# xbpeng/DeepTerrainRL

Measured on AMD Instinct MI355X. Metric: env-steps/sec (batched rollout) dog/slopes_mixed, higher is better.
Workload: dtype f64

## Files before the change

### deepterrainrl_amd/csrc/dtrl_kernel.h

```cpp
#pragma once
#include "dtrl_types.h"
#include <cmath>

#if defined(__HIPCC__)
#include <hip/hip_runtime.h>
#define DTRL_HD __host__ __device__
#define DTRL_HD_INLINE __host__ __device__ __forceinline__
#define DTRL_HD_NOINLINE __host__ __device__ __attribute__((noinline))
#else
#define DTRL_HD
#define DTRL_HD_INLINE inline
#define DTRL_HD_NOINLINE inline
#endif

#if defined(__HIP_DEVICE_COMPILE__)
#define LANES_BEGIN { const int lane = static_cast<int>(threadIdx.x);
#define LANES_END } ::dtrl::env_sync();
#else
#define LANES_BEGIN for (int lane = 0; lane < ::dtrl::kGroup; ++lane) {
#define LANES_END }
#endif

#if defined(__HIP_DEVICE_COMPILE__) && defined(DTRL_PROFILE)
#define PROF_T0() const unsigned long long prof_t0_ = __builtin_readcyclecounter()
#define PROF_ADD(ws, id) do { if (threadIdx.x == 0) (ws).prof[id] += __builtin_readcyclecounter() - prof_t0_; } while (0)
#define PROF_NOW() __builtin_readcyclecounter()
#define PROF_ADD_SINCE(ws, id, t0) do { if (threadIdx.x == 0) (ws).prof[id] += __builtin_readcyclecounter() - (t0); } while (0)
#define PROF_COUNT(ws, id) do { if (threadIdx.x == 0) (ws).prof[id] += 1; } while (0)
#else
#define PROF_T0() do {} while (0)
#define PROF_ADD(ws, id) do {} while (0)
#define PROF_NOW() 0ull
#define PROF_ADD_SINCE(ws, id, t0) do { (void)(t0); } while (0)
#define PROF_COUNT(ws, id) do {} while (0)
#endif

namespace dtrl {

#if defined(__HIP_DEVICE_COMPILE__)
#ifndef DTRL_WAVE_SYNC
#define DTRL_WAVE_SYNC 1
#endif
#if DTRL_WAVE_SYNC && !defined(__GFX9__)
#error "env_sync(): wavefront-scope fences are only a barrier when the 64-thread workgroup is ONE wavefront (GFX9 / CDNA: wave64). On a wave32 target the workgroup is two waves: build with -DDTRL_WAVE_SYNC=0 (ADVICE r4)"
#endif
__device__ __forceinline__ void env_sync()
{
#if DTRL_WAVE_SYNC
	static_assert(kGroup == 64, "env_sync(): one wavefront per env");
	__builtin_amdgcn_fence(__ATOMIC_RELEASE, "wavefront");
	__builtin_amdgcn_wave_barrier();
	__builtin_amdgcn_fence(__ATOMIC_ACQUIRE, "wavefront");
#else
	__syncthreads();
#endif
}
#else
inline void env_sync() {}
#endif

enum ProfSection { kProfFK, kProfMass, kProfBias, kProfFact, kProfDetect, kProfRows, kProfFsub, kProfDelassus, kProfPgs, kProfFinish, kProfCtrl, kProfAction, kProfFrameIO, kProfTotal, kProfRowsSum, kProfSubsteps, kProfP1, kProfP2, kProfP3, kProfP4, kProfR0, kProfR1_6, kProfR7_12, kProfR13_18, kProfR19_24, kProfT0, kProfT1_6, kProfT7_12, kProfT13_18, kProfT19_24, kProfNNConv, kProfNNFcTerr, kProfNNRest, kProfNNEvals, kProfC_Fsm, kProfC_Feedback, kProfC_PdSetup, kProfC_PdSolve, kProfC_Grav, kProfC_Tail, kProfMax };

struct HotModel {
	int32_t L, D, char_type, n_pairs;
	int32_t warm_start;
	int32_t parent[kMaxL], depth[kMaxL], col[kMaxL];
	int8_t pair_l[kMaxPairs], pair_k[kMaxPairs];
	alignas(4) int8_t path[kMaxL][kMaxDepth];
	uint32_t sub_mask[kMaxL];
	uint32_t anc_mask[kMaxL];
	real attach[kMaxL][2], lim_lo[kMaxL], lim_hi[kMaxL];
	real body_attach[kMaxL][2];
	real mass[kMaxL], inertia[kMaxL], sub_mass[kMaxL];
	int32_t n_cpairs;
	int8_t cp_a[kMaxCP], cp_b[kMaxCP];
	float cp_half[kMaxL][2];
	float cp_root_bt[2];
};

struct DevBuffers {
	EnvState* st;
	GroundRec* gr;
	EnvStatus* status;
	real* poli_state;
	real* tup_s0;
	real* tup_a;
	real* nn_out;
	float* tuple_rows;
	uint32_t* tuple_flags;
	int32_t* tuple_env;
	int32_t* tuple_count;
	int32_t tuple_cap;
	int32_t S, A, W;
	int32_t model_D;
	int32_t model_topo;
	unsigned long long* prof;
	const int32_t* env_list;
	int32_t reset_listed;
	GroundGen* gen;
	const TerrainCfg* tcfg;
	DistRec* dist_ring; int32_t* dist_count; int32_t dist_cap;
	const GroundRec* gr_stage; int32_t* stage_slot;
	const float* weights;
	const real* in_off; const real* in_scale; const real* out_off; const real* out_scale;
	NetDesc net;
};

constexpr int kZStride = kMaxD + 1;
struct WSBase {
	HotModel M;
	EnvState st;
	real phi[kMaxL], cs[kMaxL], sn[kMaxL], w[kMaxL];
	real px[kMaxL], py[kMaxL], cx[kMaxL], cy[kMaxL];
	real vpx[kMaxL], vpy[kMaxL], vcx[kMaxL], vcy[kMaxL];
	real fx[kMaxL], fy[kMaxL], fn[kMaxL];
	real mcx[kMaxL], mcy[kMaxL], Io[kMaxL];
	real sfs[3][kMaxL];
	union {
		struct { real bx[kMaxL], by[kMaxL], ux[kMaxL], uy[kMaxL], gx[kMaxL], gy[kMaxL]; };
		struct { real sm[kMaxL], smx[kMaxL], smy[kMaxL], sI[kMaxL]; };
	};
	real dinv[kMaxD];
	real b[kMaxD];
	real u[kMaxD];
	int32_t R, n_pts_active;
	int32_t row_kind[kMaxRows], row_link[kMaxRows];
	int8_t row_link2[kMaxRows];
	real row_x[kMaxRows], row_y[kMaxRows], row_dx[kMaxRows], row_dy[kMaxRows], row_tgt[kMaxRows];
	uint16_t row_id[kMaxRows];
	real wv[kMaxRows], rinv[kMaxRows];
	real dl;
	union {
		real Z[kMaxRows + 1][kZStride];
		struct {
			real z0_[kZStride];
			real basis[kMaxD][4];
			real tau_g[kMaxD];
			real kpv[kMaxD], kdv[kMaxD], kdm[kMaxD], perr[kMaxD], verr[kMaxD];
		};
	};
	real red[8];
	int32_t flag_update_action, flag_new_cycle, flag_misc;
	int32_t cost;
#if defined(DTRL_PROFILE)
	unsigned long long prof[kProfMax];
#endif
};
struct WSRef : WSBase {
	real H[kMaxD][kMaxD + 1];
	union {
		real A[kMaxRows][kMaxRows + 1];
		struct {
			real pt_x[kMaxPts], pt_y[kMaxPts], pt_depth[kMaxPts], pt_nx[kMaxPts], pt_ny[kMaxPts];
			int32_t pt_active[kMaxPts];
		};
	};
};
constexpr int kPackedA = kMaxRows * (kMaxRows + 1) / 2;
constexpr int kMassTab = kMaxL * (kMaxDepth + 2);
struct WSFast : WSBase {
	real Apk[kPackedA > kMassTab ? kPackedA : kMassTab];
};


DTRL_HD_INLINE real fmadd(real a, real b, real c) { return __builtin_fma(a, b, c); }
DTRL_HD_INLINE void sincos_r(real x, real* s, real* c)
{
#if defined(DTRL_REAL_F32)
	sincosf(x, s, c);
#else
	sincos(x, s, c);
#endif
}
#if defined(__HIP_DEVICE_COMPILE__)
typedef real v4r_t __attribute__((ext_vector_type(4)));
__device__ __forceinline__ v4r_t mfma_16x16x4(real a, real b, v4r_t acc)
{
#if defined(DTRL_REAL_F32)
	return __builtin_amdgcn_mfma_f32_16x16x4f32(a, b, acc, 0, 0, 0);
#else
	return __builtin_amdgcn_mfma_f64_16x16x4f64(a, b, acc, 0, 0, 0);
#endif
}
__device__ __forceinline__ constexpr int mfma_row(int r, int g)
{
#if defined(DTRL_REAL_F32)
	return 4 * g + r;
#else
	return 4 * r + g;
#endif
}
#endif
DTRL_HD_INLINE real fast_recip(real x)
{
#if defined(__HIP_DEVICE_COMPILE__)
	real r = __builtin_amdgcn_rcp(x);
	r = __builtin_fma(__builtin_fma(-x, r, 1.0), r, r);
	r = __builtin_fma(__builtin_fma(-x, r, 1.0), r, r);
	return r;
#else
	return 1.0 / x;
#endif
}
DTRL_HD_INLINE real fast_rsqrt(real x)
{
#if defined(__HIP_DEVICE_COMPILE__)
	real r = __builtin_amdgcn_rsq(x);
	const real hx = 0.5 * x;
	r = __builtin_fma(__builtin_fma(-hx * r, r, 0.5), r, r);
	r = __builtin_fma(__builtin_fma(-hx * r, r, 0.5), r, r);
	return r;
#else
	return 1.0 / sqrt(x);
#endif
}

DTRL_HD_INLINE real clamp_turn_rate(real v, int dof, real h)
{
	if (dof < 2) return v;
	const real vmax = kMaxTurnPerSubstep / h;
	return v > vmax ? vmax : (v < -vmax ? -vmax : v);
}
DTRL_HD inline real wrap_pi(real a)
{
	const real pi = 3.14159265358979323846, two_pi = 6.283185307179586476925286766559;
	real r = fmod(a + pi, two_pi);
	if (r < 0) r += two_pi;
	return r - pi;
}

DTRL_HD inline uint64_t rng_mix(uint64_t x)
{
	x += 0x9E3779B97F4A7C15ULL;
	x = (x ^ (x >> 30)) * 0xBF58476D1CE4E5B9ULL;
	x = (x ^ (x >> 27)) * 0x94D049BB133111EBULL;
	return x ^ (x >> 31);
}
struct Rng {
	uint64_t key; uint64_t* ctr;
	DTRL_HD real uniform() { uint64_t z = rng_mix(key + (*ctr) * 0xD1342543DE82EF95ULL); ++(*ctr); return static_cast<real>(z >> 11) * (1.0 / 9007199254740992.0); }
	DTRL_HD real uniform(real mn, real mx) { return mn + uniform() * (mx - mn); }
	DTRL_HD int rand_int(int mn, int mx) { if (mn == mx) return mn; int r = mn + static_cast<int>(uniform() * (mx - mn)); return r >= mx ? mx - 1 : r; }
	DTRL_HD bool flip() { return uniform() < 0.5; }
	DTRL_HD real normal(real mean, real stdev)
	{
		real u1 = 1.0 - uniform(), u2 = uniform();
		return mean + stdev * sqrt(-2.0 * log(u1)) * cos(6.283185307179586476925286766559 * u2);
	}
};
DTRL_HD inline Rng make_rng(const RunParams& rp, int env, uint64_t* ctr)
{
	Rng r; r.key = rng_mix(rp.rng_seed ^ rng_mix(static_cast<uint64_t>(rp.env_id_base + env))); r.ctr = ctr; return r;
}

struct GroundHdr { real mx0, o0, o1, sc0, sc1; int w0, w1; };
DTRL_HD_INLINE GroundHdr ground_header(const GroundRec& g)
{
	GroundHdr h;
	h.mx0 = g.max_x[0]; h.w0 = g.w[0]; h.w1 = g.w[1];
	h.o0 = g.origin_x[0]; h.o1 = g.origin_x[1]; h.sc0 = g.scale_x[0]; h.sc1 = g.scale_x[1];
	return h;
}
DTRL_HD_INLINE real sample_ground(const GroundRec& g, const GroundHdr& gh, real x, real* slope, int* oi, int* oj, int* oseg)
{
	const real mx0 = gh.mx0;
	const int w0 = gh.w0, w1 = gh.w1;
	const real o0 = gh.o0, o1 = gh.o1, sc0 = gh.sc0, sc1 = gh.sc1;
	const int seg = (x >= mx0) ? 1 : 0;
	const int w = seg ? w1 : w0;
	const real scale = seg ? sc1 : sc0;
	const real tol = 0.0001;
	real c = x - (seg ? o1 : o0);
	c /= scale;
	c += ((w - 1) * 0.5);
	if (c > -tol && c < w - 1 + tol) { c = c < 0.0 ? 0.0 : (c > w - 1.0 ? w - 1.0 : c); }
	c = !(c > 0.0) ? 0.0 : (c > w - 1.0 ? w - 1.0 : c);
	int i = static_cast<int>(c);
	int j = (i + 1 < w - 1) ? i + 1 : w - 1;
	real lerp = c - i;
	const real inv_run = fast_recip(scale * ((j - i) > 0 ? (j - i) : 1));
	real a = g.data[seg][i];
	real b = g.data[seg][j];
	if (slope) *slope = (j == i) ? 0.0 : (b - a) * inv_run;
	if (oi) *oi = i;
	if (oj) *oj = j;
	if (oseg) *oseg = seg;
	return (1 - lerp) * a + lerp * b;
}
DTRL_HD_INLINE real sample_ground(const GroundRec& g, real x, real* slope, int* oi, int* oj, int* oseg)
{
	const GroundHdr gh = ground_header(g);
	return sample_ground(g, gh, x, slope, oi, oj, oseg);
}

static_assert(kMaxDepth % 4 == 0, "path rows are read as 32-bit words");
template <class W>
DTRL_HD_INLINE uint32_t path_word(const W& ws, int j, int t)
{
#if defined(__HIP_DEVICE_COMPILE__)
	return reinterpret_cast<const uint32_t*>(&ws.M.path[j][0])[t];
#else
	uint32_t w; __builtin_memcpy(&w, &ws.M.path[j][4 * t], 4); return w;
#endif
}
template <class W>
DTRL_HD inline void kin_dyn_terms(W& ws)
{
	PROF_T0();
	LANES_BEGIN
	if (lane < ws.M.L) {
		const int j = lane;
		const int dep = ws.M.depth[j];
		real phi = 0, w = 0;
		const uint32_t pw[kMaxDepth / 4] = {path_word(ws, j, 0), path_word(ws, j, 1), path_word(ws, j, 2)};
#pragma unroll
		for (int k = 0; k < kMaxDepth; ++k) {
			const int a = (k <= dep) ? static_cast<int>((pw[k / 4] >> (8 * (k % 4))) & 0xffu) : 0;
			const real qa = ws.st.q[a + 2], wa = ws.st.qd[a + 2];
			const real on = (k <= dep) ? 1.0 : 0.0;
			phi = fmadd(qa, on, phi); w = fmadd(wa, on, w);
		}
		ws.phi[j] = phi; ws.w[j] = w;
		real s, c; sincos_r(phi, &s, &c);
		ws.cs[j] = c; ws.sn[j] = s;
	}
	LANES_END
	PROF_ADD(ws, kProfP1);
	LANES_BEGIN
	if (lane < ws.M.L) {
		const int j = lane;
		const int pa = ws.M.parent[j];
		real rx = 0, ry = 0, ux = 0, uy = 0, gx = 0, gy = 0;
		if (pa >= 0) {
			const real c = ws.cs[pa], s = ws.sn[pa], wp = ws.w[pa];
			rx = c * ws.M.attach[j][0] - s * ws.M.attach[j][1];
			ry = s * ws.M.attach[j][0] + c * ws.M.attach[j][1];
			ux = -(wp * ry); uy = wp * rx;
			const real w2 = wp * wp;
			gx = -(w2 * rx); gy = -(w2 * ry);
		}
		ws.bx[j] = rx; ws.by[j] = ry; ws.ux[j] = ux; ws.uy[j] = uy; ws.gx[j] = gx; ws.gy[j] = gy;
	}
	LANES_END
	PROF_ADD(ws, kProfP2);
	LANES_BEGIN
	if (lane < ws.M.L) {
		const int j = lane;
		const int dep = ws.M.depth[j];
		const real ax0 = 0, ay0 = -kGravityY;
		real px = 0, py = 0, vx = ws.st.qd[0], vy = ws.st.qd[1], ax = 0, ay = 0;
		const uint32_t pw[kMaxDepth / 4] = {path_word(ws, j, 0), path_word(ws, j, 1), path_word(ws, j, 2)};
#pragma unroll
		for (int k = 1; k < kMaxDepth; ++k) {
			const int a = (k <= dep) ? static_cast<int>((pw[k / 4] >> (8 * (k % 4))) & 0xffu) : 0;
			const real rx = ws.bx[a], ry = ws.by[a], dux = ws.ux[a], duy = ws.uy[a], dgx = ws.gx[a], dgy = ws.gy[a];
			const real on = (k <= dep) ? 1.0 : 0.0;
			px = fmadd(rx, on, px); py = fmadd(ry, on, py); vx = fmadd(dux, on, vx); vy = fmadd(duy, on, vy); ax = fmadd(dgx, on, ax); ay = fmadd(dgy, on, ay);
		}
		ws.px[j] = px; ws.py[j] = py; ws.vpx[j] = vx; ws.vpy[j] = vy;
		const real c = ws.cs[j], s = ws.sn[j], wj = ws.w[j];
		const real rx = c * ws.M.body_attach[j][0] - s * ws.M.body_attach[j][1];
		const real ry = s * ws.M.body_attach[j][0] + c * ws.M.body_attach[j][1];
		const real cx = px + rx, cy = py + ry;
		ws.cx[j] = cx; ws.cy[j] = cy;
// ... 1580 lines not shown
```

### deepterrainrl_amd/csrc/dtrl_kernel_fast.h

```cpp
#pragma once
#include "dtrl_kernel.h"
#include "dtrl_topo.h"
#include <type_traits>

#if defined(__HIP_DEVICE_COMPILE__)

#if !DTRL_WAVE_SYNC
#error "dtrl_kernel_fast.h: the register-resident path is ONE wavefront per env by construction (v_readlane broadcasts, ballots, and LDS read-then-write sequences such as warm_match_fast() that rely on a wave's LDS operations completing in issue order). -DDTRL_WAVE_SYNC=0 builds the lane-phase reference path only (ADVICE r5)"
#endif

namespace dtrl {

__device__ __forceinline__ int lane_id() { return static_cast<int>(threadIdx.x); }
#if defined(DTRL_REAL_F32)
#define DTRL_VFMA "v_fma_f32"
#define DTRL_VMOV "v_mov_b32"
#else
#define DTRL_VFMA "v_fma_f64"
#define DTRL_VMOV "v_mov_b64"
#endif
__device__ __forceinline__ real bcast(real v, int src)
{
#if defined(DTRL_REAL_F32)
	return __int_as_float(__builtin_amdgcn_readlane(__float_as_int(v), src));
#else
	int lo = __builtin_amdgcn_readlane(__double2loint(v), src);
	int hi = __builtin_amdgcn_readlane(__double2hiint(v), src);
	return __hiloint2double(hi, lo);
#endif
}

template <int D>
__device__ __forceinline__ void mass_row(WSFast& ws, real (&h)[D])
{
	constexpr int Lk = D - 2;
	constexpr int kTab = Lk * (Lk + 5) / 2;
	constexpr int kFill = (kTab + 1) & ~1;
	static_assert(kFill <= static_cast<int>(sizeof(ws.Apk) / sizeof(real)), "mass table does not fit the packed-matrix storage");
	const int d = static_cast<int>(threadIdx.x);
	const int l = d >= 2 ? d - 2 : 0;
	const bool hinge = d >= 2 && d < D;
	real* T = ws.Apk;
	{
		struct alignas(2 * sizeof(real)) real2 { real x, y; };
		real2* T2 = reinterpret_cast<real2*>(T);
		const real2 z2 = {0.0, 0.0};
#pragma unroll
		for (int e = 0; e < (kFill / 2 + kGroup - 1) / kGroup; ++e) if (d + e * kGroup < kFill / 2) T2[d + e * kGroup] = z2;
	}
	env_sync();
	if (hinge) {
		const int base = l * (l + 5) / 2;
		const real m = ws.sm[l], mx = ws.smx[l], my = ws.smy[l];
		T[base] = -(my - m * ws.py[l]);
		T[base + 1] = (mx - m * ws.px[l]);
	}
	const int n_pairs = ws.M.n_pairs;
#pragma unroll 2
	for (int e = lane_id(); e < n_pairs; e += kGroup) {
		const int pl = ws.M.pair_l[e], pk = ws.M.pair_k[e];
		const int a = ws.M.path[pl][pk];
		const real m = ws.sm[pl], mx = ws.smx[pl], my = ws.smy[pl], I = ws.sI[pl];
		const real plx = ws.px[pl], ply = ws.py[pl];
		const real pax = ws.px[a], pay = ws.py[a];
		T[pl * (pl + 5) / 2 + 2 + a] = I - ((plx + pax) * mx + (ply + pay) * my) + m * (plx * pax + ply * pay);
	}
	env_sync();
	const real M0 = ws.sm[0];
	const real* Tl = T + (d < D ? d : 0);
	h[0] = (d == 0) ? M0 : 0.0;
	h[1] = (d == 1) ? M0 : 0.0;
#pragma unroll
	for (int c = 2; c < D; ++c) h[c] = Tl[(c - 2) * (c + 3) / 2];
	env_sync();
}

template <int B, int E, class F>
__device__ __forceinline__ void static_for(F&& f)
{
	if constexpr (B < E) { f(std::integral_constant<int, B>{}); static_for<B + 1, E>(f); }
}
template <int B, int E, class F>
__device__ __forceinline__ void static_for_down(F&& f)
{
	if constexpr (B < E) { f(std::integral_constant<int, E - 1>{}); static_for_down<B, E - 1>(f); }
}
template <int J>
__device__ __forceinline__ void fnma_lanes_ge(real& acc, real a, real b)
{
	unsigned long long sv, m;
	asm("s_lshl_b64 %2, -1, %5\n\ts_and_saveexec_b64 %1, %2\n\t" DTRL_VFMA " %0, -%3, %4, %0\n\ts_mov_b64 exec, %1"
	    : "+v"(acc), "=&s"(sv), "=&s"(m) : "v"(a), "s"(b), "n"(J) : "scc");
}
template <int J>
__device__ __forceinline__ void fnma_lanes_ge(real (&acc)[1], real a, const real (&b)[1]) { fnma_lanes_ge<J>(acc[0], a, b[0]); }
template <int J>
__device__ __forceinline__ void fnma_lanes_ge(real (&acc)[2], real a, const real (&b)[2])
{
	unsigned long long sv, m;
	asm("s_lshl_b64 %3, -1, %7\n\ts_and_saveexec_b64 %2, %3\n\t" DTRL_VFMA " %0, -%4, %5, %0\n\t" DTRL_VFMA " %1, -%4, %6, %1\n\ts_mov_b64 exec, %2"
	    : "+v"(acc[0]), "+v"(acc[1]), "=&s"(sv), "=&s"(m) : "v"(a), "s"(b[0]), "s"(b[1]), "n"(J) : "scc");
}
template <int J>
__device__ __forceinline__ void fnma_lanes_ge(real (&acc)[4], real a, const real (&b)[4])
{
	unsigned long long sv, m;
	asm("s_lshl_b64 %5, -1, %11\n\ts_and_saveexec_b64 %4, %5\n\t" DTRL_VFMA " %0, -%6, %7, %0\n\t" DTRL_VFMA " %1, -%6, %8, %1\n\t"
	    "" DTRL_VFMA " %2, -%6, %9, %2\n\t" DTRL_VFMA " %3, -%6, %10, %3\n\ts_mov_b64 exec, %4"
	    : "+v"(acc[0]), "+v"(acc[1]), "+v"(acc[2]), "+v"(acc[3]), "=&s"(sv), "=&s"(m)
	    : "v"(a), "s"(b[0]), "s"(b[1]), "s"(b[2]), "s"(b[3]), "n"(J) : "scc");
}
template <int I>
__device__ __forceinline__ void fnma_lanes_lt(real& acc, real a, real b)
{
	unsigned long long sv, m;
	asm("s_bfm_b64 %2, %5, 0\n\ts_and_saveexec_b64 %1, %2\n\t" DTRL_VFMA " %0, -%3, %4, %0\n\ts_mov_b64 exec, %1"
	    : "+v"(acc), "=&s"(sv), "=&s"(m) : "v"(a), "s"(b), "n"(I) : "scc");
}
template <int K>
__device__ __forceinline__ void mov_lane_eq(real& dst, real src)
{
	unsigned long long sv, m;
	asm("s_lshl_b64 %2, 1, %4\n\ts_and_saveexec_b64 %1, %2\n\t" DTRL_VMOV " %0, %3\n\ts_mov_b64 exec, %1"
	    : "+v"(dst), "=&s"(sv), "=&s"(m) : "v"(src), "n"(K) : "scc");
}
template <int I>
__device__ __forceinline__ void mov_lanes_lt(real& dst, real src)
{
	unsigned long long sv, m;
	asm("s_bfm_b64 %2, %4, 0\n\ts_and_saveexec_b64 %1, %2\n\t" DTRL_VMOV " %0, %3\n\ts_mov_b64 exec, %1"
	    : "+v"(dst), "=&s"(sv), "=&s"(m) : "v"(src), "n"(I) : "scc");
}
template <int J>
__device__ __forceinline__ void mov_lanes_ge(real& dst, real src)
{
	unsigned long long sv, m;
	asm("s_lshl_b64 %2, -1, %4\n\ts_and_saveexec_b64 %1, %2\n\t" DTRL_VMOV " %0, %3\n\ts_mov_b64 exec, %1"
	    : "+v"(dst), "=&s"(sv), "=&s"(m) : "v"(src), "n"(J) : "scc");
}

template <int I>
__device__ __forceinline__ void fnma_lanes_lt(real (&acc)[1], real a, const real (&b)[1]) { fnma_lanes_lt<I>(acc[0], a, b[0]); }
template <int I>
__device__ __forceinline__ void fnma_lanes_lt(real (&acc)[2], real a, const real (&b)[2])
{
	unsigned long long sv, m;
	asm("s_bfm_b64 %3, %7, 0\n\ts_and_saveexec_b64 %2, %3\n\t" DTRL_VFMA " %0, -%4, %5, %0\n\t" DTRL_VFMA " %1, -%4, %6, %1\n\ts_mov_b64 exec, %2"
	    : "+v"(acc[0]), "+v"(acc[1]), "=&s"(sv), "=&s"(m) : "v"(a), "s"(b[0]), "s"(b[1]), "n"(I) : "scc");
}
template <int I>
__device__ __forceinline__ void fnma_lanes_lt(real (&acc)[4], real a, const real (&b)[4])
{
	unsigned long long sv, m;
	asm("s_bfm_b64 %5, %11, 0\n\ts_and_saveexec_b64 %4, %5\n\t" DTRL_VFMA " %0, -%6, %7, %0\n\t" DTRL_VFMA " %1, -%6, %8, %1\n\t"
	    "" DTRL_VFMA " %2, -%6, %9, %2\n\t" DTRL_VFMA " %3, -%6, %10, %3\n\ts_mov_b64 exec, %4"
	    : "+v"(acc[0]), "+v"(acc[1]), "+v"(acc[2]), "+v"(acc[3]), "=&s"(sv), "=&s"(m)
	    : "v"(a), "s"(b[0]), "s"(b[1]), "s"(b[2]), "s"(b[3]), "n"(I) : "scc");
}

template <class Topo>
__device__ __forceinline__ real factorize_regs(WSFast& ws, real (&h)[Topo::L + 2])
{
	constexpr int D = Topo::L + 2;
	const int lane = static_cast<int>(threadIdx.x);
	real dinv = 0;
	static_for_down<1, D>([&](auto kc) {
		constexpr int k = decltype(kc)::value;
		const real dk = bcast(h[k], k);
		const real ak = h[k];
		const real rk = fast_recip(dk);
		mov_lane_eq<k>(dinv, rk);
		const real lik = ak * rk;
		static_for_down<0, k>([&](auto jc) {
			constexpr int j = decltype(jc)::value;
			if constexpr (dof_coupled<Topo>(j, k)) h[j] = fmadd(-lik, bcast(ak, j), h[j]);
		});
		mov_lanes_lt<k>(h[k], lik);
	});
	{ const real r0 = fast_recip(h[0]); if (lane == 0) dinv = r0; }
	real* S = ws.Apk;
#pragma unroll
	for (int k = 1; k < D; ++k) if (lane < k) S[k * (k - 1) / 2 + lane] = h[k];
	env_sync();
	const int base = lane * (lane - 1) / 2;
#pragma unroll
	for (int k = 0; k < D - 1; ++k) if (lane > k && lane < D) h[k] = S[base + k];
	env_sync();
	return dinv;
}
template <int D>
__device__ __forceinline__ real usolve_regs(const real (&h)[D], real z)
{
	static_for_down<1, D>([&](auto kc) {
		constexpr int k = decltype(kc)::value;
		const real zk = bcast(z, k);
		fnma_lanes_lt<k>(z, h[k], zk);
	});
	return z;
}
template <int D, int NR>
__device__ __forceinline__ void usolve_regs_n(const real (&h)[D], real (&z)[NR])
{
	static_for_down<1, D>([&](auto kc) {
		constexpr int k = decltype(kc)::value;
		real zk[NR];
#pragma unroll
		for (int j = 0; j < NR; ++j) zk[j] = bcast(z[j], k);
		fnma_lanes_lt<k>(z, h[k], zk);
	});
}
template <int D>
__device__ __forceinline__ real utsolve_regs(const real (&h)[D], real u)
{
	static_for<0, D - 1>([&](auto kc) {
		constexpr int k = decltype(kc)::value;
		const real uk = bcast(u, k);
		fnma_lanes_ge<k + 1>(u, h[k], uk);
	});
	return u;
}

static_assert((kMaxPts + kGroup - 1) / kGroup == 3, "written for 3 sample points per lane");
struct ContactPts { PtVal p0, p1, p2; unsigned long long m0, m1, m2;  unsigned long long f0, f1, f2;  };
__device__ __forceinline__ int opaque_lane()
{
	int lane = static_cast<int>(threadIdx.x);
	asm volatile("" : "+v"(lane));
	return lane;
}
__device__ __forceinline__ unsigned link_field(unsigned long long m0, unsigned long long m1, unsigned long long m2, int link)
{
	const int b = link * kPtsPerLink, word = b >> 6, off = b & 63;
	unsigned long long lo = m0, hi = m1;
	if (word == 1) { lo = m1; hi = m2; }
	if (word == 2) { lo = m2; hi = 0ull; }
	unsigned long long bits = lo >> off;
	if (off + kPtsPerLink > 64) bits |= hi << (64 - off);
	return static_cast<unsigned>(bits & ((1ull << kPtsPerLink) - 1ull));
}
constexpr real kNoPoint = -1.0e30;
__device__ __noinline__ unsigned link_cap_drop_mask(WSFast& ws, real d0, real d1, real d2)
{
	const int lane = opaque_lane();
	const int npts = ws.M.L * kPtsPerLink;
	real* S = ws.Apk;
	if (lane < npts) S[lane] = d0;
	if (lane + kGroup < npts) S[lane + kGroup] = d1;
	if (lane + 2 * kGroup < npts) S[lane + 2 * kGroup] = d2;
	env_sync();
	auto over = [&](real d, int pt) -> unsigned {
		if (!(d > kNoPoint)) return 0u;
		const int base = (pt / kPtsPerLink) * kPtsPerLink;
		int rank = 0;
		for (int k = 0; k < kPtsPerLink; ++k) { const int o = base + k; const real od = S[o]; rank += (o != pt && (od > d || (od == d && o < pt))) ? 1 : 0; }
		return rank >= kMaxPtsPerLink ? 1u : 0u;
	};
	const unsigned m = over(d0, lane) | (over(d1, lane + kGroup) << 1) | (over(d2, lane + 2 * kGroup) << 2);
	env_sync();
	return m;
}
template <bool kFlags>
__device__ __forceinline__ ContactPts eval_points(WSFast& ws, const DevModel& gm, const GroundRec& g)
{
	const int lane = opaque_lane();
	const int npts = ws.M.L * kPtsPerLink;
	ContactPts c;
	PtVal z; z.x = 0; z.y = 0; z.depth = 0; z.nx = 0; z.ny = 0; z.active = 0; z.near = 0;
	c.p0 = z; c.p1 = z; c.p2 = z;
	if (lane < npts) c.p0 = contact_point_eval<kFlags>(ws, gm, g, lane);
	if (lane + kGroup < npts) c.p1 = contact_point_eval<kFlags>(ws, gm, g, lane + kGroup);
	if (lane + 2 * kGroup < npts) c.p2 = contact_point_eval<kFlags>(ws, gm, g, lane + 2 * kGroup);
	c.f0 = 0; c.f1 = 0; c.f2 = 0;
	if (kFlags) { c.f0 = __ballot(c.p0.near); c.f1 = __ballot(c.p1.near); c.f2 = __ballot(c.p2.near); }
	c.m0 = __ballot(c.p0.active); c.m1 = __ballot(c.p1.active); c.m2 = __ballot(c.p2.active);
	if ((c.m0 | c.m1 | c.m2) != 0ull) {
		const int many = (lane < ws.M.L) && __popc(link_field(c.m0, c.m1, c.m2, lane)) > kMaxPtsPerLink;
		if (__builtin_expect(__ballot(many) != 0ull, 0)) {
			const unsigned drop = link_cap_drop_mask(ws, c.p0.active ? c.p0.depth : kNoPoint, c.p1.active ? c.p1.depth : kNoPoint, c.p2.active ? c.p2.depth : kNoPoint);
			if (drop & 1u) c.p0.active = 0;
			if (drop & 2u) c.p1.active = 0;
			if (drop & 4u) c.p2.active = 0;
			c.m0 = __ballot(c.p0.active); c.m1 = __ballot(c.p1.active); c.m2 = __ballot(c.p2.active);
		}
	}
	return c;
}
__device__ __noinline__ unsigned row_cap_drop_mask(WSFast& ws, real d0, real d1, real d2, int cap)
{
	const int lane = opaque_lane();
	const int npts = ws.M.L * kPtsPerLink;
	real* S = ws.Apk;
	if (lane < npts) S[lane] = d0;
	if (lane + kGroup < npts) S[lane + kGroup] = d1;
	if (lane + 2 * kGroup < npts) S[lane + 2 * kGroup] = d2;
	env_sync();
	auto over = [&](real d, int pt) -> unsigned {
		if (!(d > kNoPoint)) return 0u;
		int rank = 0;
		for (int o = 0; o < npts; ++o) { const real od = S[o]; rank += (o != pt && (od > d || (od == d && o < pt))) ? 1 : 0; }
		return rank >= cap ? 1u : 0u;
	};
	const unsigned m = over(d0, lane) | (over(d1, lane + kGroup) << 1) | (over(d2, lane + 2 * kGroup) << 2);
	env_sync();
	return m;
}
__device__ __forceinline__ unsigned long long pairs_in_reach(const WSFast& ws)
{
	const int lane = static_cast<int>(threadIdx.x);
	return __ballot(lane < ws.M.n_cpairs && pair_in_reach(ws, lane));
}
constexpr int kPairCands = 2 * kPtsPerLink, kPairSlots = kGroup / kPairCands;
__device__ __noinline__ int append_pair_rows_fast(WSFast& ws, const DevModel& gm, int R, unsigned long long reach)
{
	const int lane = opaque_lane();
	const unsigned long long below = (lane == 0) ? 0ull : (~0ull >> (64 - lane));
	const int slot = lane / kPairCands, cand = lane - slot * kPairCands;
	while (reach != 0ull && R + 2 <= kMaxRows) {
		int mypr = -1;
#pragma unroll
		for (int sidx = 0; sidx < kPairSlots; ++sidx) {
			if (reach != 0ull) { const int pr = __ffsll(static_cast<long long>(reach)) - 1; reach &= reach - 1ull; if (slot == sidx) mypr = pr; }
		}
		int P = 0, Q = 0, k = 0;
		PairHit hit; hit.active = 0; hit.depth = 0; hit.x = 0; hit.y = 0; hit.nx = 0; hit.ny = 0;
		if (mypr >= 0) { pair_candidate(ws.M.cp_a[mypr], ws.M.cp_b[mypr], cand, &P, &Q, &k); hit = pair_point_eval(ws, gm, P, Q, k); }
		const unsigned long long am = __ballot(hit.active);
		if (am == 0ull) continue;
		int keep = hit.active;
		const int mine_cnt = __popcll((am >> (slot * kPairCands)) & ((1ull << kPairCands) - 1ull));
		if (__builtin_expect(__ballot(lane < kPairSlots * kPairCands && mine_cnt > kMaxPtsPerPair) != 0ull, 0)) {
			real* S = ws.Apk;
			S[lane] = hit.active ? hit.depth : -1.0;
			env_sync();
			if (hit.active) {
				int rank = 0;
				for (int o = 0; o < kPairCands; ++o) { const real od = S[slot * kPairCands + o]; rank += (o != cand && od > 0 && (od > hit.depth || (od == hit.depth && o < cand))) ? 1 : 0; }
				keep = rank < kMaxPtsPerPair;
			}
			env_sync();
		}
		const unsigned long long km = __ballot(keep);
		const int room = (kMaxRows - R) / 2;
		const int idx = __popcll(km & below);
		if (keep && idx < room) {
			const int Rw = R + 2 * idx;
			ws.row_kind[Rw] = 1; ws.row_link[Rw] = P; ws.row_link2[Rw] = static_cast<int8_t>(Q); ws.row_x[Rw] = hit.x; ws.row_y[Rw] = hit.y;
			ws.row_dx[Rw] = hit.nx; ws.row_dy[Rw] = hit.ny; ws.row_tgt[Rw] = 0;
			ws.row_id[Rw] = pair_row_id(mypr, cand, 0); ws.row_id[Rw + 1] = pair_row_id(mypr, cand, 1);
			ws.row_kind[Rw + 1] = 2; ws.row_link[Rw + 1] = P; ws.row_link2[Rw + 1] = static_cast<int8_t>(Q); ws.row_x[Rw + 1] = hit.x; ws.row_y[Rw + 1] = hit.y;
			ws.row_dx[Rw + 1] = hit.ny; ws.row_dy[Rw + 1] = -hit.nx; ws.row_tgt[Rw + 1] = 0;
		}
		int n = __popcll(km); if (n > room) n = room;
		R += 2 * n;
	}
	return R;
}
__device__ __forceinline__ void contact_bits_fast(WSFast& ws, unsigned long long m0, unsigned long long m1, unsigned long long m2)
{
	const int lane = static_cast<int>(threadIdx.x);
	int any = 0;
	if (lane < ws.M.L) any = link_field(m0, m1, m2, lane) != 0u;
	const unsigned long long lm = __ballot(any);
	if (lane == 0) ws.st.contact_bits = static_cast<uint32_t>(lm);
}
__device__ __forceinline__ void detect_contacts_fast(WSFast& ws, const DevModel& gm, const GroundRec& g)
{
	const ContactPts c = eval_points<true>(ws, gm, g);
	contact_bits_fast(ws, c.f0, c.f1, c.f2);
	env_sync();
}
__device__ __forceinline__ void emit_contact_rows(WSFast& ws, const PtVal& p, int pt, int rank, int cap, int R0, real inv_h)
{
	if (p.active && rank < cap) {
		const int R = R0 + 2 * rank;
		const int j = pt / kPtsPerLink;
		ws.row_kind[R] = 1; ws.row_link[R] = j; ws.row_link2[R] = -1; ws.row_x[R] = p.x; ws.row_y[R] = p.y;
		ws.row_dx[R] = p.nx; ws.row_dy[R] = p.ny; ws.row_tgt[R] = normal_row_target(p.depth, inv_h);
		ws.row_id[R] = ground_row_id(pt, 0); ws.row_id[R + 1] = ground_row_id(pt, 1);
		ws.row_kind[R + 1] = 2; ws.row_link[R + 1] = j; ws.row_link2[R + 1] = -1; ws.row_x[R + 1] = p.x; ws.row_y[R + 1] = p.y;
		ws.row_dx[R + 1] = p.ny; ws.row_dy[R + 1] = -p.nx; ws.row_tgt[R + 1] = 0;
	}
}
__device__ __forceinline__ void build_rows_fast(WSFast& ws, const DevModel& gm, const ContactPts& c_in, real h)
{
	ContactPts c = c_in;
	const int lane = static_cast<int>(threadIdx.x);
	const unsigned long long below = (lane == 0) ? 0ull : (~0ull >> (64 - lane));
	const real inv_h = 1.0 / h;
	int lim = 0; real tgt = 0;
	if (lane >= 1 && lane < ws.M.L && !(ws.M.lim_lo[lane] > ws.M.lim_hi[lane])) {
		const real th = ws.st.q[lane + 2];
		if (th <= ws.M.lim_lo[lane] + kLimitSlop) { lim = 1; tgt = kLimitErp * fmax(ws.M.lim_lo[lane] - th, 0.0) * inv_h; }
		else if (th >= ws.M.lim_hi[lane] - kLimitSlop) { lim = -1; tgt = kLimitErp * fmax(th - ws.M.lim_hi[lane], 0.0) * inv_h; }
	}
	const unsigned long long ml = __ballot(lim != 0);
	const int rl = __popcll(ml & below);
	int R0 = __popcll(ml); if (R0 > kMaxRows) R0 = kMaxRows;
	if (lim != 0 && rl < kMaxRows) { ws.row_kind[rl] = 0; ws.row_link[rl] = lane; ws.row_link2[rl] = -1; ws.row_dx[rl] = lim; ws.row_tgt[rl] = tgt; ws.row_id[rl] = kNoRowId; }
	const int cap = (kMaxRows - R0) / 2;
	if (__builtin_expect(__popcll(c.m0) + __popcll(c.m1) + __popcll(c.m2) > cap, 0)) {
		const unsigned drop = row_cap_drop_mask(ws, c.p0.active ? c.p0.depth : kNoPoint, c.p1.active ? c.p1.depth : kNoPoint, c.p2.active ? c.p2.depth : kNoPoint, cap);
		if (drop & 1u) c.p0.active = 0;
		if (drop & 2u) c.p1.active = 0;
		if (drop & 4u) c.p2.active = 0;
		c.m0 = __ballot(c.p0.active); c.m1 = __ballot(c.p1.active); c.m2 = __ballot(c.p2.active);
	}
	const int n0 = __popcll(c.m0), n1 = __popcll(c.m1), n2 = __popcll(c.m2);
	emit_contact_rows(ws, c.p0, lane, __popcll(c.m0 & below), cap, R0, inv_h);
	emit_contact_rows(ws, c.p1, lane + kGroup, n0 + __popcll(c.m1 & below), cap, R0, inv_h);
	emit_contact_rows(ws, c.p2, lane + 2 * kGroup, n0 + n1 + __popcll(c.m2 & below), cap, R0, inv_h);
	int nc = n0 + n1 + n2; if (nc > cap) nc = cap;
	int R = R0 + 2 * nc;
	const unsigned long long reach = pairs_in_reach(ws);
	if (__builtin_expect(reach != 0ull, 0)) R = append_pair_rows_fast(ws, gm, R, reach);
	if (lane == 0) ws.R = R;
	env_sync();
}

template <int D>
__device__ __forceinline__ void build_delassus_fast(WSFast& ws, real h, real dinv_mine)
{
	const int lane = static_cast<int>(threadIdx.x);
	const int R = ws.R;
	const int n_ent = R * (R + 1) / 2;
	if (R < 16) {
		typedef v4r_t v4d_t;
		const int g = lane >> 4, c = lane & 15;
		real jv = 0;
		if (lane < R) {
			const int sw = lane;
			if (ws.row_kind[sw] == 0) jv = ws.row_dx[sw] * ws.st.qd[ws.row_link[sw] + 2];
			else jv = row_point_jv(ws, sw);
		}
		const int zrow = c <= R ? c : 0;
		v4d_t acc = {0, 0, 0, 0};
#pragma unroll
		for (int s4 = 0; s4 < (D + 3) / 4; ++s4) {
			const int k = 4 * s4 + g;
			const bool live = k < D;
			const real z = ws.Z[zrow][live ? k : 0], dk = ws.dinv[live ? k : 0];
			const real b = live ? z : 0.0;
			const real a = live ? z * dk : 0.0;
			acc = mfma_16x16x4(a, b, acc);
		}
#pragma unroll
		for (int r = 0; r < 4; ++r) {
			const int i = mfma_row(r, g);
			if (i < R && c <= i) ws.Apk[i * (i + 1) / 2 + c] = acc[r];
			if (i < R && c == R) ws.wv[i] = acc[r];
		}
		env_sync();
		if (lane < R) ws.wv[lane] = jv + h * ws.wv[lane] - ws.row_tgt[lane];
		env_sync();
		return;
	}
	const real* di = ws.dinv;
	auto entry_rows = [](int e, int& s, int& r) {
		s = static_cast<int>((sqrtf(8.0f * e + 1.0f) - 1.0f) * 0.5f);
		while (s * (s + 1) / 2 > e) --s;
		while ((s + 1) * (s + 2) / 2 <= e) ++s;
		r = e - s * (s + 1) / 2;
	};
	{
		const bool has_e = lane < n_ent, has_w = lane < R;
		int s = 0, r = 0;
		if (has_e) entry_rows(lane, s, r);
		const int sw = has_w ? lane : 0;
		real jv = 0;
		if (has_w) {
			if (ws.row_kind[sw] == 0) jv = ws.row_dx[sw] * ws.st.qd[ws.row_link[sw] + 2];
			else jv = row_point_jv(ws, sw);
		}
		const real* zs = ws.Z[s];
		const real* zr = ws.Z[r];
		const real* zw = ws.Z[sw];
		const real* z0 = ws.Z[R];
		real a = 0, zz = 0;
#pragma unroll 4
		for (int i = 0; i < D; ++i) { a = fmadd(zs[i] * di[i], zr[i], a); zz = fmadd(zw[i] * di[i], z0[i], zz); }
		if (has_e) ws.Apk[lane] = a;
		if (has_w) ws.wv[lane] = jv + h * zz - ws.row_tgt[lane];
	}
	for (int e = lane + kGroup; e < n_ent; e += kGroup) {
		int s, r; entry_rows(e, s, r);
		const real* zs = ws.Z[s];
		const real* zr = ws.Z[r];
		real a = 0;
#pragma unroll 4
		for (int i = 0; i < D; ++i) a = fmadd(zs[i] * di[i], zr[i], a);
		ws.Apk[e] = a;
	}
	env_sync();
}

__device__ __forceinline__ real wave_shr1(real v)
{
#if defined(DTRL_REAL_F32)
	return __int_as_float(__builtin_amdgcn_update_dpp(0, __float_as_int(v), 0x138, 0xf, 0xf, false));
#else
	const int lo = __builtin_amdgcn_update_dpp(0, __double2loint(v), 0x138, 0xf, 0xf, false);
	const int hi = __builtin_amdgcn_update_dpp(0, __double2hiint(v), 0x138, 0xf, 0xf, false);
	return __hiloint2double(hi, lo);
#endif
}
template <int r, int K>
__device__ __forceinline__ void pgs_rows_load(real (&a)[K], const WSFast& ws, int lane, bool mine, int R)
{
	if constexpr (r < K) {
		if (r < R) {
			const int mx = lane > r ? lane : r, mn = lane < r ? lane : r;
			a[r] = ws.Apk[mine ? mx * (mx + 1) / 2 + mn : 0];
			pgs_rows_load<r + 1, K>(a, ws, lane, mine, R);
		}
	}
}
template <int r, int K, int kEnd>
__device__ __forceinline__ void pgs_rows_sweep(const real (&a)[K], const WSFast& ws, real& w, real& lam, real rinv, bool tang, bool mine, unsigned long long actR, int lane, int R, real a_pref)
{
	if constexpr (r < kEnd) {
		if (r < R) {
			real a_sr;
			if constexpr (r < K) a_sr = a[r]; else a_sr = a_pref;
			real a_nx = 0.0;
			if constexpr (r + 1 >= K && r + 1 < kEnd) {
				constexpr int rn = r + 1;
				const int mx = lane > rn ? lane : rn, mn = lane < rn ? lane : rn;
				a_nx = ws.Apk[(mine && rn < R) ? mx * (mx + 1) / 2 + mn : 0];
			}
			if ((actR >> r) & 1ull) {
				const real lim = kMu * wave_shr1(lam);
				const real lo = tang ? -lim : 0.0, hi = tang ? lim : __builtin_huge_val();
				const real nl = fmin(fmax(fmadd(-w, rinv, lam), lo), hi);
				const real dl = bcast(nl - lam, r);
				if (lane == r) lam = nl;
				w = fmadd(a_sr, dl, w);
			}
			pgs_rows_sweep<r + 1, K, kEnd>(a, ws, w, lam, rinv, tang, mine, actR, lane, R, a_nx);
		}
	}
}
template <bool kFric, int r, int K, int kEnd>
__device__ __forceinline__ void pgs_rows_pass(const real (&a)[K], const WSFast& ws, real& w, real& lam, real rinv, real lo, real hi, bool mine, unsigned long long rows, int lane, int R, real a_pref)
{
	if constexpr (r < kEnd) {
		if (r < R) {
			real a_sr;
			if constexpr (r < K) a_sr = a[r]; else a_sr = a_pref;
			real a_nx = 0.0;
			if constexpr (r + 1 >= K && r + 1 < kEnd) {
				constexpr int rn = r + 1;
				const int mx = lane > rn ? lane : rn, mn = lane < rn ? lane : rn;
				a_nx = ws.Apk[(mine && rn < R) ? mx * (mx + 1) / 2 + mn : 0];
			}
			if ((rows >> r) & 1ull) {
				real nl = fmadd(-w, rinv, lam);
				if constexpr (kFric) nl = fmin(fmax(nl, lo), hi); else nl = fmax(nl, 0.0);
				const real dl = bcast(nl - lam, r);
				if (lane == r) lam = nl;
				w = fmadd(a_sr, dl, w);
			}
			pgs_rows_pass<kFric, r + 1, K, kEnd>(a, ws, w, lam, rinv, lo, hi, mine, rows, lane, R, a_nx);
		}
	}
}
template <int r, int K, int kEnd>
__device__ __forceinline__ void pgs_rows_warm(const real (&a)[K], const WSFast& ws, real& w, real lam, bool mine, unsigned long long nz, int lane, int R)
{
	if constexpr (r < kEnd) {
		if (r < R) {
			if ((nz >> r) & 1ull) {
				real a_sr;
				if constexpr (r < K) a_sr = a[r];
				else { const int mx = lane > r ? lane : r, mn = lane < r ? lane : r; a_sr = ws.Apk[mine ? mx * (mx + 1) / 2 + mn : 0]; }
				w = fmadd(a_sr, bcast(lam, r), w);
			}
			pgs_rows_warm<r + 1, K, kEnd>(a, ws, w, lam, mine, nz, lane, R);
		}
	}
}
__device__ __forceinline__ void warm_match_fast(WSFast& ws)
{
	const int lane = opaque_lane();
	const int R = ws.R, Rp = ws.st.ws_R;
	if (R == 0) { if (Rp != 0 && lane == 0) ws.st.ws_R = 0; return; }
	int id = kNoRowId;
	if (lane < R) id = ws.row_id[lane];
	real l0 = 0.0;
	if (ws.M.warm_start != 0 && Rp > 0) {
		int hit = -1;
		for (int p = 0; p < Rp; ++p) hit = (ws.st.ws_id[p] == id) ? p : hit;
		if (id < kFirstPairRowId && hit >= 0) l0 = kWarmFactor * ws.st.ws_lam[hit];
	}
	if (lane < R) { ws.st.ws_lam[lane] = l0; ws.st.ws_id[lane] = static_cast<uint16_t>(id); }
	if (lane == 0) ws.st.ws_R = R;
}
template <int kPgsRegRows, bool kTailInSweep>
__device__ __forceinline__ void pgs_solve_fast(WSFast& ws)
{
	const int lane = opaque_lane();
	const int R = ws.R;
	const bool mine = lane < R;
	real w = mine ? ws.wv[lane] : 0.0;
	real rinv = 0.0;
	if (mine) { const real ass = ws.Apk[lane * (lane + 3) / 2]; rinv = (ass >= 1e-12) ? 1.0 / ass : 0.0; }
	real lam = (mine && rinv != 0.0) ? ws.st.ws_lam[lane] : 0.0;
	const bool tang = mine && ws.row_kind[lane] == 2;
	const unsigned long long act = __ballot(rinv != 0.0);
	const bool warm = ws.M.warm_start != 0;
	const unsigned long long tmask = __ballot(tang);
	const unsigned long long nz_l0 = __ballot(lam != 0.0);
	const bool any_l0 = nz_l0 != 0ull;
	if (kTailInSweep || R <= kPgsRegRows) {
		real a[kPgsRegRows];
		pgs_rows_load<0, kPgsRegRows>(a, ws, lane, mine, R);
		const unsigned long long actR = act & ((R < 64) ? ((1ull << R) - 1ull) : ~0ull);
		constexpr int kEnd = kTailInSweep ? kMaxRows : kPgsRegRows;
		if (any_l0) pgs_rows_warm<0, kPgsRegRows, kEnd>(a, ws, w, lam, mine, nz_l0, lane, R);
		const unsigned long long pass0 = warm ? (actR & ~tmask) : actR, pass1 = actR & tmask;
		if (warm) {
			constexpr bool kPrefetch = kTailInSweep && kPgsRegRows < kMaxRows;
			const int end0 = (kPrefetch || pass0 == 0ull) ? R : 64 - __builtin_clzll(pass0);
#pragma unroll 1
			for (int it = 0; it < kPgsIters; ++it) {
				if (pass0 != 0ull) pgs_rows_pass<false, 0, kPgsRegRows, kEnd>(a, ws, w, lam, rinv, 0.0, 0.0, mine, pass0, lane, end0, 0.0);
				const real ln = wave_shr1(lam);
				const real lim = kMu * ln;
				const unsigned long long rows = pass1 & __ballot(tang && ln > kHoldEps);
				if (rows != 0ull) pgs_rows_pass<true, 0, kPgsRegRows, kEnd>(a, ws, w, lam, rinv, -lim, lim, mine, rows, lane, kPrefetch ? R : 64 - __builtin_clzll(rows), 0.0);
			}
		} else {
#pragma unroll 1
			for (int it = 0; it < kPgsIters; ++it) pgs_rows_sweep<0, kPgsRegRows, kEnd>(a, ws, w, lam, rinv, tang, mine, actR, lane, R, 0.0);
		}
		if (mine) ws.st.ws_lam[lane] = lam;
		env_sync();
		return;
	}
	const int tri = lane * (lane + 1) / 2;
	const real inf = __builtin_huge_val();
	if (any_l0) for (int r = 0; r < R; ++r) if ((nz_l0 >> r) & 1ull) { const int mx = lane > r ? lane : r, mn = lane < r ? lane : r; w = fmadd(ws.Apk[mine ? mx * (mx + 1) / 2 + mn : 0], bcast(lam, r), w); }
	real a_nx = mine ? ws.Apk[tri] : 0.0;
	const unsigned long long actR = act & ((R < 64) ? ((1ull << R) - 1ull) : ~0ull);
	if (warm) {
		const unsigned long long pass0 = actR & ~tmask, pass1 = actR & tmask;
		for (int it = 0; it < kPgsIters; ++it) {
			for (int r = 0; r < R; ++r) {
				const real a_sr = a_nx;
				const int rn = (r + 1 < R) ? r + 1 : 0;
				{ const int mx = lane > rn ? lane : rn, mn = lane < rn ? lane : rn; a_nx = ws.Apk[mine ? mx * (mx + 1) / 2 + mn : 0]; }
				if (!((pass0 >> r) & 1ull)) continue;
				const real nl = fmax(fmadd(-w, rinv, lam), 0.0);
				const real dl = bcast(nl - lam, r);
				if (lane == r) lam = nl;
				w = fmadd(a_sr, dl, w);
			}
			const real ln = wave_shr1(lam);
			const real lim = kMu * ln;
			const unsigned long long rows = pass1 & __ballot(tang && ln > kHoldEps);
			for (int r = 0; r < R; ++r) {
				const real a_sr = a_nx;
				const int rn = (r + 1 < R) ? r + 1 : 0;
				{ const int mx = lane > rn ? lane : rn, mn = lane < rn ? lane : rn; a_nx = ws.Apk[mine ? mx * (mx + 1) / 2 + mn : 0]; }
				if (!((rows >> r) & 1ull)) continue;
				const real nl = fmin(fmax(fmadd(-w, rinv, lam), -lim), lim);
				const real dl = bcast(nl - lam, r);
				if (lane == r) lam = nl;
				w = fmadd(a_sr, dl, w);
			}
		}
	} else {
		for (int it = 0; it < kPgsIters; ++it) {
			for (int r = 0; r < R; ++r) {
				const real a_sr = a_nx;
				const int rn = (r + 1 < R) ? r + 1 : 0;
				{ const int mx = lane > rn ? lane : rn, mn = lane < rn ? lane : rn; a_nx = ws.Apk[mine ? mx * (mx + 1) / 2 + mn : 0]; }
				if (!((act >> r) & 1ull)) continue;
				const real lim = kMu * wave_shr1(lam);
				const real lo = tang ? -lim : 0.0, hi = tang ? lim : inf;
				const real nl = fmin(fmax(fmadd(-w, rinv, lam), lo), hi);
				const real dl = bcast(nl - lam, r);
				if (lane == r) lam = nl;
				w = fmadd(a_sr, dl, w);
			}
		}
	}
	if (mine) ws.st.ws_lam[lane] = lam;
	env_sync();
}

template <class Topo>
struct FastPath {
	static constexpr int D = Topo::L + 2;
	static __device__ void substep(WSFast& ws, const DevModel& gm, const GroundRec& g, real h, bool kin_valid)
	{
		const int lane = static_cast<int>(threadIdx.x);
#if defined(DTRL_PROFILE)
		const unsigned long long prof_sub_t0 = __builtin_readcyclecounter();
#endif
		if (!kin_valid) { PROF_T0(); kin_dyn_terms(ws); PROF_ADD(ws, kProfFK); }
		const int rows_ready = kin_valid ? ws.n_pts_active : -1;
		if (rows_ready >= 0) {
			if (lane == 0) { ws.R = rows_ready; ws.n_pts_active = -1; }
			env_sync();
		} else {
			ContactPts cp;
			{ PROF_T0(); cp = eval_points<false>(ws, gm, g); PROF_ADD(ws, kProfDetect); }
			{ PROF_T0(); build_rows_fast(ws, gm, cp, h); PROF_ADD(ws, kProfRows); }
		}
		{ PROF_T0(); warm_match_fast(ws); PROF_ADD(ws, kProfRows); }
		real hrow[D];
		{ PROF_T0(); mass_row<D>(ws, hrow); PROF_ADD(ws, kProfMass); }
		real dinv;
		{ PROF_T0(); dinv = factorize_regs<Topo>(ws, hrow); PROF_ADD(ws, kProfFact); }
		const int R = ws.R;
		if (lane == 0) ws.cost += 8 + R;
		{
			PROF_T0();
			const bool hinge = lane >= 2 && lane < D;
			const real mypx = hinge ? ws.px[lane - 2] : 0.0, mypy = hinge ? ws.py[lane - 2] : 0.0;
			const uint32_t mysub = hinge ? ws.M.sub_mask[lane - 2] : 0u;
			real rhs0 = (lane < D) ? (ws.st.tau[lane] - ws.b[lane]) : 0.0;
			if (__builtin_expect(ws.st.pert_on != 0, 0)) { if (lane < D) rhs0 += perturb_gen_force(ws, lane); }
			auto rhs_of = [&](int r) -> real {
				if (r >= R) return rhs0;
				const int kind = ws.row_kind[r], link = ws.row_link[r];
				const real dx = ws.row_dx[r];
				if (kind == 0) return (lane == link + 2) ? dx : 0.0;
				const real dy = ws.row_dy[r], x = ws.row_x[r], y = ws.row_y[r];
				const int link2 = ws.row_link2[r];
				if (lane == 0) return link2 < 0 ? dx : 0.0;
				if (lane == 1) return link2 < 0 ? dy : 0.0;
				const int on = static_cast<int>((mysub >> link) & 1u) - (link2 < 0 ? 0 : static_cast<int>((mysub >> link2) & 1u));
				if (on == 0) return 0.0;
				const real jr = dx * (-(y - mypy)) + dy * (x - mypx);
				return on > 0 ? jr : -jr;
			};
			int r0 = 0;
			for (; r0 + 4 <= R + 1; r0 += 4) {
				real z[4] = {rhs_of(r0), rhs_of(r0 + 1), rhs_of(r0 + 2), rhs_of(r0 + 3)};
				usolve_regs_n<D, 4>(hrow, z);
#pragma unroll
				for (int j = 0; j < 4; ++j) if (lane < D) ws.Z[r0 + j][lane] = z[j];
			}
			if (r0 + 2 <= R + 1) {
				real z[2] = {rhs_of(r0), rhs_of(r0 + 1)};
				usolve_regs_n<D, 2>(hrow, z);
				if (lane < D) { ws.Z[r0][lane] = z[0]; ws.Z[r0 + 1][lane] = z[1]; }
				r0 += 2;
			}
			if (r0 <= R) {
				real z[1] = {rhs_of(r0)};
				usolve_regs_n<D, 1>(hrow, z);
				if (lane < D) ws.Z[r0][lane] = z[0];
			}
			if (lane < D) ws.dinv[lane] = dinv;
			env_sync();
			PROF_ADD(ws, kProfFsub);
		}
		if (R > 0) {
			{ PROF_T0(); build_delassus_fast<D>(ws, h, dinv); PROF_ADD(ws, kProfDelassus); }
			{ PROF_T0(); pgs_solve_fast<Topo::kPgsRegRows, Topo::kPgsTailInSweep>(ws); PROF_ADD(ws, kProfPgs); }
		}
		{
			PROF_T0();
			real u = 0;
			if (lane < D) {
				real s = h * ws.Z[R][lane];
				for (int r = 0; r < R; ++r) s = fmadd(ws.Z[r][lane], ws.st.ws_lam[r], s);
				u = s * dinv;
			}
			u = utsolve_regs<D>(hrow, u);
			if (lane < D) { const real v = clamp_turn_rate(ws.st.qd[lane] + u, lane, h); ws.st.qd[lane] = v; ws.st.q[lane] += h * v; }
			env_sync();
			PROF_ADD(ws, kProfFinish);
		}
#if defined(DTRL_PROFILE)
		if (threadIdx.x == 0) { ws.prof[kProfRowsSum] += R; ws.prof[kProfSubsteps] += 1; const int bk = R == 0 ? 0 : (R <= 6 ? 1 : (R <= 12 ? 2 : (R <= 18 ? 3 : 4))); ws.prof[kProfR0 + bk] += 1; ws.prof[kProfT0 + bk] += __builtin_readcyclecounter() - prof_sub_t0; }
#endif
	}
	static __device__ void pd_solve(WSFast& ws, real dt)
	{
		const int lane = static_cast<int>(threadIdx.x);
		real hrow[D];
		mass_row<D>(ws, hrow);
		const real add = (lane < D) ? dt * ws.kdm[lane] : 0.0;
#pragma unroll
		for (int k = 0; k < D; ++k) if (lane == k) hrow[k] += add;
		const real dinv = factorize_regs<Topo>(ws, hrow);
		real z = (lane < D) ? ws.u[lane] : 0.0;
		z = usolve_regs<D>(hrow, z);
		real u = z * dinv;
		u = utsolve_regs<D>(hrow, u);
		env_sync();
		if (lane < D) ws.u[lane] = u;
		if (lane == 0) ws.R = 0;
		env_sync();
	}
	static __device__ void contacts(WSFast& ws, const DevModel& gm, const GroundRec& g, real h)
	{
		const ContactPts cp = eval_points<true>(ws, gm, g);
		contact_bits_fast(ws, cp.f0, cp.f1, cp.f2);
		build_rows_fast(ws, gm, cp, h);
		if (threadIdx.x == 0) ws.n_pts_active = ws.R;
		env_sync();
	}
};

}
#endif
```

Baseline: 17.87 million.

## Solve contact-row triangular systems one row per lane instead of across lanes

The old path solved each contact row's right-hand side across lanes, one DOF per lane, using readlane broadcasts for every column, in batches of 4, 2 and 1 rows. When R is at least kFsubRowsMinR (default 1), the new path writes the RHS rows to LDS, then has each lane own one row and do a serial back-substitution. It loads only the topology-coupled entries of the packed factor from ws.Apk, software-prefetched one column ahead with sched barriers. This removes the broadcast chains and gains parallelism across rows, at the cost of more per-lane registers (acc[D] plus the packed factor), LDS traffic, and idle lanes when R is small. It also adds profiling sections bucketed by row count.

```diff
diff --git a/deepterrainrl_amd/csrc/dtrl_kernel.h b/deepterrainrl_amd/csrc/dtrl_kernel.h
--- a/deepterrainrl_amd/csrc/dtrl_kernel.h
+++ b/deepterrainrl_amd/csrc/dtrl_kernel.h
@@ -59,7 +59,7 @@
 inline void env_sync() {}
 #endif
 
-enum ProfSection { kProfFK, kProfMass, kProfBias, kProfFact, kProfDetect, kProfRows, kProfFsub, kProfDelassus, kProfPgs, kProfFinish, kProfCtrl, kProfAction, kProfFrameIO, kProfTotal, kProfRowsSum, kProfSubsteps, kProfP1, kProfP2, kProfP3, kProfP4, kProfR0, kProfR1_6, kProfR7_12, kProfR13_18, kProfR19_24, kProfT0, kProfT1_6, kProfT7_12, kProfT13_18, kProfT19_24, kProfNNConv, kProfNNFcTerr, kProfNNRest, kProfNNEvals, kProfC_Fsm, kProfC_Feedback, kProfC_PdSetup, kProfC_PdSolve, kProfC_Grav, kProfC_Tail, kProfMax };
+enum ProfSection { kProfFK, kProfMass, kProfBias, kProfFact, kProfDetect, kProfRows, kProfFsub, kProfDelassus, kProfPgs, kProfFinish, kProfCtrl, kProfAction, kProfFrameIO, kProfTotal, kProfRowsSum, kProfSubsteps, kProfP1, kProfP2, kProfP3, kProfP4, kProfR0, kProfR1_6, kProfR7_12, kProfR13_18, kProfR19_24, kProfT0, kProfT1_6, kProfT7_12, kProfT13_18, kProfT19_24, kProfNNConv, kProfNNFcTerr, kProfNNRest, kProfNNEvals, kProfC_Fsm, kProfC_Feedback, kProfC_PdSetup, kProfC_PdSolve, kProfC_Grav, kProfC_Tail, kProfFsubR0, kProfFsubR1_6, kProfFsubR7_12, kProfFsubR13_18, kProfFsubR19_24, kProfMax };
 
 struct HotModel {
 	int32_t L, D, char_type, n_pairs;
diff --git a/deepterrainrl_amd/csrc/dtrl_kernel_fast.h b/deepterrainrl_amd/csrc/dtrl_kernel_fast.h
--- a/deepterrainrl_amd/csrc/dtrl_kernel_fast.h
+++ b/deepterrainrl_amd/csrc/dtrl_kernel_fast.h
@@ -208,6 +208,44 @@
 		for (int j = 0; j < NR; ++j) zk[j] = bcast(z[j], k);
 		fnma_lanes_lt<k>(z, h[k], zk);
 	});
+}
+template <class Topo>
+constexpr int first_update_col(int i)
+{
+	for (int k = Topo::L + 1; k > i; --k) if (dof_coupled<Topo>(i, k)) return k;
+	return 0;
+}
+template <class Topo, int kAhead = 1>
+__device__ __forceinline__ void usolve_rows(WSFast& ws, int R)
+{
+	constexpr int D = Topo::L + 2;
+	const int lane = static_cast<int>(threadIdx.x);
+	if (lane > R) return;
+	real* z = ws.Z[lane];
+	const real* U = ws.Apk;
+	real acc[D], u[D * (D - 1) / 2];
+	auto fetch = [&](auto kc) {
+		constexpr int k = decltype(kc)::value;
+		static_for<0, k>([&](auto ic) {
+			constexpr int i = decltype(ic)::value;
+			if constexpr (dof_coupled<Topo>(i, k)) u[k * (k - 1) / 2 + i] = U[k * (k - 1) / 2 + i];
+			if constexpr (first_update_col<Topo>(i) == k) acc[i] = z[i];
+		});
+		if constexpr (first_update_col<Topo>(k) == 0) acc[k] = z[k];
+	};
+	static_for_down<D - kAhead, D>(fetch);
+	static_for_down<1, D>([&](auto kc) {
+		constexpr int k = decltype(kc)::value;
+		__builtin_amdgcn_sched_barrier(0);
+		if constexpr (k - kAhead >= 1) fetch(std::integral_constant<int, k - kAhead>{});
+		const real zk = acc[k];
+		if constexpr (first_update_col<Topo>(k) != 0) z[k] = zk;
+		static_for_down<0, k>([&](auto ic) {
+			constexpr int i = decltype(ic)::value;
+			if constexpr (dof_coupled<Topo>(i, k)) acc[i] = fmadd(-u[k * (k - 1) / 2 + i], zk, acc[i]);
+		});
+	});
+	z[0] = acc[0];
 }
 template <int D>
 __device__ __forceinline__ real utsolve_regs(const real (&h)[D], real u)
@@ -688,6 +726,11 @@
 	env_sync();
 }
 
+#ifndef DTRL_FSUB_ROWS_MIN_R
+#define DTRL_FSUB_ROWS_MIN_R 1
+#endif
+constexpr int kFsubRowsMinR = DTRL_FSUB_ROWS_MIN_R;
+
 template <class Topo>
 struct FastPath {
 	static constexpr int D = Topo::L + 2;
@@ -735,27 +778,40 @@
 				const real jr = dx * (-(y - mypy)) + dy * (x - mypx);
 				return on > 0 ? jr : -jr;
 			};
-			int r0 = 0;
-			for (; r0 + 4 <= R + 1; r0 += 4) {
-				real z[4] = {rhs_of(r0), rhs_of(r0 + 1), rhs_of(r0 + 2), rhs_of(r0 + 3)};
-				usolve_regs_n<D, 4>(hrow, z);
-#pragma unroll
-				for (int j = 0; j < 4; ++j) if (lane < D) ws.Z[r0 + j][lane] = z[j];
-			}
-			if (r0 + 2 <= R + 1) {
-				real z[2] = {rhs_of(r0), rhs_of(r0 + 1)};
-				usolve_regs_n<D, 2>(hrow, z);
-				if (lane < D) { ws.Z[r0][lane] = z[0]; ws.Z[r0 + 1][lane] = z[1]; }
-				r0 += 2;
-			}
-			if (r0 <= R) {
-				real z[1] = {rhs_of(r0)};
-				usolve_regs_n<D, 1>(hrow, z);
-				if (lane < D) ws.Z[r0][lane] = z[0];
+			if (R < kFsubRowsMinR) {
+				int r0 = 0;
+				if constexpr (kFsubRowsMinR >= 4) {
+					for (; r0 + 4 <= R + 1; r0 += 4) {
+						real z[4] = {rhs_of(r0), rhs_of(r0 + 1), rhs_of(r0 + 2), rhs_of(r0 + 3)};
+						usolve_regs_n<D, 4>(hrow, z);
+#pragma unroll
+						for (int j = 0; j < 4; ++j) if (lane < D) ws.Z[r0 + j][lane] = z[j];
+					}
+				}
+				if constexpr (kFsubRowsMinR >= 2) {
+					if (r0 + 2 <= R + 1) {
+						real z[2] = {rhs_of(r0), rhs_of(r0 + 1)};
+						usolve_regs_n<D, 2>(hrow, z);
+						if (lane < D) { ws.Z[r0][lane] = z[0]; ws.Z[r0 + 1][lane] = z[1]; }
+						r0 += 2;
+					}
+				}
+				if (r0 <= R) {
+					real z[1] = {rhs_of(r0)};
+					usolve_regs_n<D, 1>(hrow, z);
+					if (lane < D) ws.Z[r0][lane] = z[0];
+				}
+			} else {
+				for (int r = 0; r <= R; ++r) { const real v = rhs_of(r); if (lane < D) ws.Z[r][lane] = v; }
+				env_sync();
+				usolve_rows<Topo>(ws, R);
 			}
 			if (lane < D) ws.dinv[lane] = dinv;
 			env_sync();
 			PROF_ADD(ws, kProfFsub);
+#if defined(DTRL_PROFILE)
+			PROF_ADD(ws, kProfFsubR0 + (R == 0 ? 0 : (R <= 6 ? 1 : (R <= 12 ? 2 : (R <= 18 ? 3 : 4)))));
+#endif
 		}
 		if (R > 0) {
 			{ PROF_T0(); build_delassus_fast<D>(ws, h, dinv); PROF_ADD(ws, kProfDelassus); }
```

New measurement: 18.84 million (median of 6 runs). +5.4%, better.
